# TaliMotzkin/GroupNet

Hardware: AMD Instinct MI355X
Metric: scenes/sec GroupNet MS-HGNN forward, NBA N=11 B=512, 1/2/4/8 MI355X (higher is better)
Workload: dtype f32

## Files before the change

groupnet_amd/_lib.py:

```python
from __future__ import annotations

import ctypes
import os
import threading

import torch

_HERE = os.path.dirname(os.path.abspath(__file__))
LIB_PATH = os.environ.get("GROUPNET_HIP_LIB") or os.path.join(_HERE, "libgroupnet_hip.so")
ABI_VERSION = 34

GN_OK = 0
GN_ERR_K_RANGE = -3

_P = ctypes.c_void_p
_I = ctypes.c_int
_F = ctypes.c_float
_SZ = ctypes.c_size_t
_U64 = ctypes.c_ulonglong


def addr(t) -> int:
    return 0 if t is None else t.data_ptr()


# ... 107 lines not shown
    "gn_listall_incidence_f32": (_I, [_P, _P, _I, _I, _I, _P]),
    "gn_affinity_topk_f32": (_I, [_P, _P, ctypes.POINTER(_P), ctypes.POINTER(_I), _I, _I, _I, _I,
                                  ctypes.POINTER(BlockExtras), _P]),
    "gn_affinity_topk_bf16": (_I, [_P, _P, ctypes.POINTER(_P), ctypes.POINTER(_I), _I, _I, _I, _I,
                                   ctypes.POINTER(BlockExtras), _P]),
    "gn_packed_elems": (_SZ, [_I, _I]),
    "gn_pack_linear_f32": (_I, [_P, _P, _I, _I, _I, _I, _P]),
    "gn_split_bf16_f32": (_I, [_P, _P, _I, _I, _P]),
    "gn_split_bf16_batch_f32": (_I, [_P, _I, _I, _I, _P]),
    "gn_pack_segments_f32": (_I, [_P, _I, _I, _P]),
    "gn_node_mlp_f32": (_I, [ctypes.POINTER(NodeGroup), _I, _I, _P]),
    "gn_node_mlp_bf16": (_I, [ctypes.POINTER(NodeGroup), _I, _I, _P]),
    "gn_node_mlp_affinity_f32": (_I, [ctypes.POINTER(NodeGroup), _I, _I, ctypes.POINTER(AffinityJob), _P]),
    "gn_node_mlp_affinity_bf16": (_I, [ctypes.POINTER(NodeGroup), _I, _I, ctypes.POINTER(AffinityJob), _P]),
    "gn_affinity_tail_lds_limit": (_SZ, []),
    "gn_node2edge_f32": (_I, [ctypes.POINTER(N2EGroup), _I, _I, _I, _P]),
    "gn_node2edge_bf16": (_I, [ctypes.POINTER(N2EGroup), _I, _I, _I, _P]),
    "gn_edge_mlp_gumbel_f32": (_I, [ctypes.POINTER(EdgeGroup), _I, _F, _U64, _P, _P]),
    "gn_edge_mlp_gumbel_bf16": (_I, [ctypes.POINTER(EdgeGroup), _I, _F, _U64, _P, _P]),
    "gn_agg_gather_f32": (_I, [ctypes.POINTER(GatherGroup), _I, _I, _I, _P]),
    "gn_agg_gather_bf16": (_I, [ctypes.POINTER(GatherGroup), _I, _I, _I, _P]),
    "gn_agg_mlp_f32": (_I, [ctypes.POINTER(AggGroup), _I, _P]),
    "gn_agg_mlp_bf16": (_I, [ctypes.POINTER(AggGroup), _I, _P]),
    "gn_node_linear_f32": (_I, [_P, _P, _P, _P, _I, _I, _P]),
    "gn_agg_scatter_f32": (_I, [ctypes.POINTER(ScatterGroup), _I, _I, _I, _F, _P]),
    "gn_agg_scatter_bf16": (_I, [ctypes.POINTER(ScatterGroup), _I, _I, _I, _F, _P]),
    "gn_mlp2_f32": (_I, [ctypes.POINTER(Mlp2Group), _I, _I, _I, _I, _I, _I, _I, _F, _P]),
    "gn_mlp2_bf16": (_I, [ctypes.POINTER(Mlp2Group), _I, _I, _I, _I, _I, _I, _I, _F, _P]),
    "gn_gemm_f32": (_I, [_P, _P, _P, _I, _I, _I, _I, _I, _I, _I, _I, _P, _P, _I, _I, _F, _F, _P]),
    "gn_gemm_grouped_f32": (_I, [ctypes.POINTER(GemmDesc), _I, _P]),
    "gn_typed_bwd_f32": (_I, [_P, _P, _P, _I, _P, _P, _P, ctypes.c_longlong, _I, _I, _P]),
    "gn_axpby2d_f32": (_I, [_P, _I, _P, _I, ctypes.c_longlong, _I, _F, _F, _P]),
    "gn_gumbel_ef_f32": (_I, [_P, _P, _P, ctypes.c_longlong, _I, _I, _I, _F, _I, _P]),
    "gn_gumbel_bwd_f32": (_I, [_P, _P, _P, _P, _P, ctypes.c_longlong, _I, _I, _F, _I, _P]),
# ... 51 lines not shown
```

groupnet_amd/csrc/gn_common.hpp:

```cpp
#pragma once
#include <hip/hip_runtime.h>
#include <stdint.h>
#include <stdlib.h>

#include "../../include/groupnet_hip.h"

#define GN_WAVE 64

typedef float f32x16 __attribute__((ext_vector_type(16)));
typedef float f32x4 __attribute__((ext_vector_type(4)));

static inline bool gn_aligned16(const void* p) { return (reinterpret_cast<uintptr_t>(p) & 15u) == 0; }

static inline int gn_check_launch() { return hipGetLastError() == hipSuccess ? GN_OK : GN_ERR_LAUNCH; }

#define GN_REQUIRE_PTR(p) \
  do {                    \
    if ((p) == nullptr) return GN_ERR_NULL; \
  } while (0)
#define GN_REQUIRE_ALIGNED(p) \
  do {                        \
    if (!gn_aligned16(p)) return GN_ERR_ALIGN; \
  } while (0)

__device__ __forceinline__ int gn_uniform(int v) { return __builtin_amdgcn_readfirstlane(v); }

__device__ __forceinline__ float gn_half_sum(float v) {
#pragma unroll
  for (int m = 16; m >= 1; m >>= 1) v += __shfl_xor(v, m, GN_WAVE);
  return v;
}
__device__ __forceinline__ float gn_wave_sum(float v) {
#pragma unroll
  for (int m = 32; m >= 1; m >>= 1) v += __shfl_xor(v, m, GN_WAVE);
  return v;
}
__device__ __forceinline__ float gn_wave_max(float v) {
#pragma unroll
  for (int m = 32; m >= 1; m >>= 1) v = fmaxf(v, __shfl_xor(v, m, GN_WAVE));
  return v;
// ... 98 lines not shown
```

groupnet_amd/csrc/gn_graph.hip:

```cpp
#include "gn_mlp_common.hpp"
#include "gn_affinity.hpp"

namespace {

constexpr int kBlock = 256;
constexpr int kN2EU = 4;
constexpr size_t kLdsBudget = 128 * 1024;

__device__ __forceinline__ bool beats(float vj, int j, float vc, int c) {
  const bool nj = vj != vj, nc = vc != vc;
  if (nj || nc) return (nj && !nc) || (nj && nc && j < c);
  return vj > vc || (vj == vc && j < c);
}

template <typename T>
__device__ __forceinline__ void emit_incidence(const float* row, int N, int b, int i, int c, const ScaleList& sl) {
  T* H_cat = reinterpret_cast<T*>(sl.H_cat);
  const float v = row[c];
  int rank = 0;
  for (int j = 0; j < N; ++j) rank += beats(row[j], j, v, c) ? 1 : 0;
  for (int s = 0; s < sl.n; ++s) {
    if (sl.k[s] == N) {
      if (i == 0) {
        sl.H[s][(size_t)b * N + c] = 1.f;
// ... 903 lines not shown
#pragma unroll
    for (int l = 0; l < 4; ++l) {
      const unsigned long long gidx = blk * 4 + l;
      if (gidx >= offset && gidx - offset < n) U[gidx - offset] = gn_philox_to_uniform(c[l]);
    }
  }
}

inline int capped_grid(long long work_items, int per_block, int cap = 256 * 16) {
  long long g = (work_items + per_block - 1) / per_block;
  return (int)(g < 1 ? 1 : (g > cap ? cap : g));
}

}

extern "C" int gn_abi_version(void) { return 34; }

extern "C" const char* gn_strerror(int code) {
  switch (code) {
    case GN_OK: return "ok";
    case GN_ERR_NULL: return "null pointer";
    case GN_ERR_SHAPE: return "unsupported or non-positive size";
    case GN_ERR_K_RANGE: return "selected index k out of range";
    case GN_ERR_ALIGN: return "pointer not 16-byte aligned";
    case GN_ERR_LAUNCH: return "kernel launch failed";
    case GN_ERR_LDS: return "tile does not fit in LDS";
    default: return "unknown error";
  }
}

extern "C" int gn_affinity_f32(const float* f, float* corr, int B, int N, int D, gn_stream_t stream) {
// ... 369 lines not shown
```

groupnet_amd/csrc/gn_mlp_bf16.hpp:

```cpp
#pragma once
#include "gn_mlp_common.hpp"
#include "gn_affinity.hpp"

#include <type_traits>

namespace {

constexpr int kOccP1 = 2;

template <int P>
struct Parts {
  bf16x8 p[P];
};

typedef float f32x8 __attribute__((ext_vector_type(8)));
__device__ __forceinline__ bf16x8 cvt_half(const f32x16& v, int hf) {
  f32x8 h;
#pragma unroll
  for (int jj = 0; jj < 8; ++jj) h[jj] = v[8 * hf + jj];
  return __builtin_convertvector(h, bf16x8);
}

typedef _Float16 f16x8 __attribute__((ext_vector_type(8)));
typedef _Float16 f16x2 __attribute__((ext_vector_type(2)));
// ... 62 lines not shown
constexpr int kMfmaPerSub = P == 3 ? 6 : (P == 2 ? 3 : 1);

template <int P, typename F>
__device__ __forceinline__ void run_with_fallback(F body) {
  ovf_t ovf = {0ull, 0};
  if constexpr (P == 2) {
    body(std::integral_constant<int, 2>{}, ovf);
    if (!__syncthreads_or(ovf.mask != 0ull || ovf.wf != 0)) return;
    ovf = {0ull, 0};
    body(std::integral_constant<int, 3>{}, ovf);
  } else {
    body(std::integral_constant<int, P>{}, ovf);
  }
}
__device__ __forceinline__ int image_flag(const void* image, int substeps) {
  return *reinterpret_cast<const int*>(reinterpret_cast<const char*>(image) + (size_t)substeps * 2 * 1024);
}
template <int P>
__device__ __forceinline__ const void* pick_image(const void* x, const void* h) { return P == 2 ? h : x; }

template <int P>
__device__ __forceinline__ void mfma_substep(const f32x4 (&w)[P], const Parts<P>& x, f32x16& acc) {
  if constexpr (P == 3) {
    const bf16x8 w1 = __builtin_bit_cast(bf16x8, w[0]);
    const bf16x8 w2 = __builtin_bit_cast(bf16x8, w[1]);
    const bf16x8 w3 = __builtin_bit_cast(bf16x8, w[2]);
    acc = __builtin_amdgcn_mfma_f32_32x32x16_bf16(w3, x.p[0], acc, 0, 0, 0);
    acc = __builtin_amdgcn_mfma_f32_32x32x16_bf16(w2, x.p[1], acc, 0, 0, 0);
    acc = __builtin_amdgcn_mfma_f32_32x32x16_bf16(w1, x.p[2], acc, 0, 0, 0);
    acc = __builtin_amdgcn_mfma_f32_32x32x16_bf16(w2, x.p[0], acc, 0, 0, 0);
    acc = __builtin_amdgcn_mfma_f32_32x32x16_bf16(w1, x.p[1], acc, 0, 0, 0);
// ... 111 lines not shown
    read_ops(s % CH + QD - 1, (s + QD - 1) % QD);
#pragma unroll
    for (int b = 0; b < RB; ++b) mfma_substep<P>(q[s % QD], x_of(b), acc_of(b));
    if constexpr (FENCE) __builtin_amdgcn_sched_barrier(0);
  }
  __device__ __forceinline__ void skip(int, int s, int n) {
#pragma unroll
    for (int p = s; p < s + n; ++p)
      if (p % CH == 0) boundary(p / CH);
    const int basec = (s + n - 1) / CH;
#pragma unroll
    for (int j = 0; j + 1 < QD; ++j) read_ops(s + n + j - basec * CH, (s + n + j) % QD);
  }
};

template <int P, int IT, int OT, int HT, bool PACKED_RELU = false, typename Stream, typename PostFn>
__device__ __forceinline__ void layer_pair(Stream& ws, int c0, int s0, const Parts<P> (&xi)[IT][2],
                                           const f32x16& hid0, const float* __restrict__ b0, int h,
                                           f32x16 (&out)[OT], ovf_t& ovf, PostFn post) {
  constexpr int NA = 2 * IT, NB = 2 * OT;
  constexpr int kMfma = NA * kMfmaPerSub<P>;
  constexpr int kValuPerPhase = P == 3 ? 96 : (P == 2 ? 84 : 40);
  constexpr int kValu = (kValuPerPhase + kMfma - 1) / kMfma;
  int pos = s0;
  f32x16 hidn = hid0;
  f32x16 bias_n;
  if (HT > 1) bias_n = load_bias_tile(b0 + 32, h);
#pragma unroll
  for (int u = 0; u < NA; ++u) {
    ws.step(c0, pos, xi[u >> 1][u & 1], hidn);
    ++pos;
  }
#pragma unroll
  for (int t = 0; t < HT; ++t) {
    f32x16 cur = hidn;
    if (t + 1 < HT) {
      hidn = bias_n;
      if (t + 2 < HT) bias_n = load_bias_tile(b0 + 32 * (t + 2), h);
    }
    post(t, cur);
    Parts<P> xh[2];
    if constexpr (PACKED_RELU) {
      make_parts_relu(cur, 0, xh[0]);
      make_parts_relu(cur, 1, xh[1]);
    } else {
      make_parts<P>(cur, 0, xh[0], ovf);
      make_parts<P>(cur, 1, xh[1], ovf);
    }
    if (t + 1 < HT) {
#pragma unroll
      for (int u = 0; u < NA; ++u) {
        ws.template step<false>(c0, pos, xi[u >> 1][u & 1], hidn);
        ++pos;
      }
#pragma unroll
      for (int i = 0; i < kMfma; ++i) {
        __builtin_amdgcn_sched_group_barrier(0x008, 1, 0);
        __builtin_amdgcn_sched_group_barrier(0x002, kValu, 0);
        if ((i % kMfmaPerSub<P>) == 0)
          __builtin_amdgcn_sched_group_barrier(Stream::CH == 1 ? 0x020 : 0x100, P, 0);
      }
    }
    __builtin_amdgcn_sched_barrier(0);
#pragma unroll
    for (int u = 0; u < NB; ++u) {
      ws.step(c0, pos, xh[u & 1], out[u >> 1]);
      ++pos;
    }
  }
}

template <typename T>
__device__ __forceinline__ void store_tile(T* __restrict__ p, const f32x16& a) {
#pragma unroll
  for (int q = 0; q < 4; ++q) {
    const f32x4 v = {a[4 * q + 0], a[4 * q + 1], a[4 * q + 2], a[4 * q + 3]};
    st4(p + 8 * q, v);
  }
// ... 82 lines not shown
#pragma unroll
    for (int oo = 0; oo < 4; ++oo) {
      const int o = o0 + o4 + oo;
      f32x16 acc = bn;
      bn = load_bias_tile(G.bA + 32 * min(o + 1, o0 + nt - 1), h);
#pragma unroll
      for (int i = 0; i < 4; ++i) ws.step(o4 * 4 / WS::CH, 4 * oo + i, xi[i >> 1][i & 1], acc);
      if (rb.live) store_tile(arow + 32 * o, acc);
    }
  }
}
template <int P>
constexpr int kRingF4For = WStream<P == 2 ? 3 : P>::kRingF4;

template <int P, typename T>
__global__ __launch_bounds__(256, 2) void node_stage_kernel(NodeTable Tb) {
  __shared__ f32x4 wring[kRingF4For<P>];
  if (Tb.aff_scenes > 0 && (int)blockIdx.x >= Tb.node_grid) {
    extern __shared__ __align__(16) float aff_lds[];
    affinity_topk_body<T>(reinterpret_cast<const T*>(Tb.aff_f), Tb.aff_corr, Tb.aff_sl, Tb.aff_N, Tb.aff_D, Tb.aff_ex,
                          (int)blockIdx.x - Tb.node_grid, aff_lds);
    return;
  }
  run_with_fallback<P>([&](auto pc, ovf_t& ovf) { node_stage_body<decltype(pc)::value, T>(Tb, wring, ovf); });
}

template <int P, typename T>
__device__ __forceinline__ void edge_x_body(const GroupTable<gn_edge_group_t>& Tb, float tau, unsigned long long seed,
                                            const unsigned long long* __restrict__ offset_dev, int pool_bytes,
                                            f32x4* wring, ovf_t& ovf) {
  using WS = WStream<P>;
  extern __shared__ __align__(16) unsigned char pool_dyn[];
  const int lwg = gn_uniform(gn_xcd_logical(Tb.xs, blockIdx.x));
  if (lwg < 0) return;
  const int gi = find_group(Tb, lwg);
  const gn_edge_group_t G = Tb.g[gi];
  const int rows = G.rows, K = G.K;
  const bool sparse = hyper_unstaged(G, 128, PoolStage<T>::kPitch * sizeof(T), pool_bytes);
  const int blk = sparse ? (wave_id() == 0 ? lwg - Tb.first_wg[gi] : (rows + 31) / 32) : (lwg - Tb.first_wg[gi]) * 4 + wave_id();
  const RowBlock rb = row_block(rows, blk);
  const int lane = rb.lane, h = rb.h;
  f32x16 in[2], z[2], lg;
  if (G.edges != nullptr) {
    load_rows<2>(reinterpret_cast<const T*>(G.edges), GN_FEAT, rb.row_ld, h, in);
  } else {
    const int nodes_max = G.pool_H == nullptr && G.sym_N > 0 ? pool_stage_nodes(128, gn_pair_count(G.pool_N), G.pool_N) : 0;
    const int r0 = (lwg - Tb.first_wg[gi]) * 128;
    if (G.pool_H != nullptr) {
      if (pool_bytes < 0)
        pooled_rows<T>(G, rb.row_ld, h, in);
      else if ((size_t)hyper_stage_nodes(128, G.pool_E, G.pool_N) * PoolStage<T>::kPitch * sizeof(T) <= (size_t)pool_bytes) {
        pooled_rows_hyper_staged<T, 1>(G, r0, min(rows - 1, r0 + 127), {rb.row_ld}, h, reinterpret_cast<T*>(pool_dyn),
                                       [&](auto, f32x16 (&p)[2]) { in[0] = p[0], in[1] = p[1]; });
      } else
        pooled_rows_hyper<T>(G, rb.row_ld, h, in);
    } else if (nodes_max > 0 && pool_bytes >= 0 && PoolStage<T>::bytes(nodes_max) <= (size_t)pool_bytes) {
      T* s_xp = reinterpret_cast<T*>(pool_dyn);
      T* s_pq = s_xp + (size_t)nodes_max * PoolStage<T>::kPitch;
      const int node0 = pool_stage_fill<T>(G, r0, min(rows - 1, r0 + 127), s_xp, s_pq);
      __syncthreads();
      pooled_rows_staged<T>(G, rb.row_ld, h, s_xp, s_pq, node0, in);
    } else {
      pooled_rows<T>(G, rb.row_ld, h, in);
    }
  }
  long long o1 = rb.row_ld, o2 = rb.row_ld;
  bool diag = true;
  if (G.sym_N > 0) {
    const int N = G.sym_N, Pn = gn_pair_count(N);
    const int b = rb.row_ld / Pn, p = rb.row_ld - b * Pn;
    int i, j;
    gn_pair_decode(p, N, i, j);
    o1 = (long long)b * N * N + i * N + j;
    o2 = (long long)b * N * N + j * N + i;
    diag = i == j;
  }
  float u1[8], u2[8];
  const unsigned long long pbase = G.philox_offset + (offset_dev ? *offset_dev : 0ull);
  const float* bi0 = G.bias;
  const float* bi1 = G.bias + 128;
  const float* bd0 = G.bias + 192;
  const float* bd1 = G.bias + 448;
  WS ws;
  const void* img = pick_image<P>(G.Wx, G.Wh);
  if constexpr (P == 2) ovf.wf |= image_flag(img, 80);
  ws.begin(img, wring, lane, wave_id(), 80 / WS::CH);
  const f32x16 hidA0 = load_bias_tile(bi0, h);
  z[0] = load_bias_tile(bi1, h);
  z[1] = load_bias_tile(bi1 + 32, h);
  Parts<P> xi[2][2];
  make_parts_tiles<P, 2>(in, xi, ovf);
  layer_pair<P, 2, 2, 4, P == 1>(ws, 0, 0, xi, hidA0, bi0, h, z, ovf, [&](int t, f32x16& hid) {
    if constexpr (P != 1) {
      relu16(hid);
      if (G.keep_z1 != nullptr && rb.live) store_tile(G.keep_z1 + (size_t)rb.row * 128 + 32 * t + 4 * h, hid);
    }
  });
  if (G.keep_z != nullptr) store_rows<2>(G.keep_z, GN_FEAT, rb.row, h, rb.live, z);
  const f32x16 hidB0 = load_bias_tile(bd0, h);
  f32x16 lgv[1];
  lgv[0] = load_bias_tile(bd1, h);
  make_parts_tiles<P, 2>(z, xi, ovf);
  layer_pair<P, 2, 1, 8, P == 1>(ws, 0, 32, xi, hidB0, bd0, h, lgv, ovf, [&](int t, f32x16& hid) {
    if constexpr (P != 1) {
      relu16(hid);
      if (G.keep_dh1 != nullptr && rb.live) store_tile(G.keep_dh1 + (size_t)rb.row * 256 + 32 * t + 4 * h, hid);
    }
  });
  lg = lgv[0];
  fetch_uniforms(G.U, pbase, seed, o1, K, h, u1);
  if (G.sym_N > 0) fetch_uniforms(G.U, pbase, seed, o2, K, h, u2);
  if (G.keep_lgf != nullptr && rb.live) store_tile(G.keep_lgf + (size_t)rb.row * 32 + 4 * h, lg);

  float facv = 0.f;
#pragma unroll
  for (int r = 0; r < 8; ++r)
    if (feat_of(r, h) == K) facv = lg[r];
  facv += __shfl_xor(facv, 32, GN_WAVE);
  const float sig = 1.f / (1.f + expf(-facv));
  float d1[8], d2[8];
  gumbel_softmax_row<P == 1>(lg, u1, K, tau, h, d1);
  if (G.sym_N > 0) gumbel_softmax_row<P == 1>(lg, u2, K, tau, h, d2);
  if (rb.live) {
    float* frow = G.edge_feat + (size_t)rb.row * K;
    T* dist = reinterpret_cast<T*>(G.dist);
    if (G.sym_N == 0) {
      T* drow = dist + (size_t)rb.row * K;
#pragma unroll
      for (int r = 0; r < 8; ++r) {
        const int f = feat_of(r, h);
        if (f < K) {
          st1(drow + f, d1[r]);
          frow[f] = sig * d1[r];
        }
      }
    } else {
#pragma unroll
      for (int r = 0; r < 8; ++r) {
        const int f = feat_of(r, h);
        if (f < K) {
          if (dist != nullptr) {
            st1(dist + (size_t)o1 * K + f, d1[r]);
            if (!diag) st1(dist + (size_t)o2 * K + f, d2[r]);
          }
          frow[f] = diag ? 2.f * (sig * d1[r]) : sig * d1[r] + sig * d2[r];
        }
      }
    }
  }
}
template <int P, typename T>
__global__ __launch_bounds__(256, P == 1 ? kOccP1 : 2) void edge_x_kernel(GroupTable<gn_edge_group_t> Tb, float tau,
                                                        unsigned long long seed,
                                                        const unsigned long long* __restrict__ offset_dev, int pool_bytes) {
  __shared__ f32x4 wring[kRingF4For<P>];
  run_with_fallback<P>([&](auto pc, ovf_t& ovf) {
    edge_x_body<decltype(pc)::value, T>(Tb, tau, seed, offset_dev, pool_bytes, wring, ovf);
  });
}

__device__ __forceinline__ void add_b2(const float* __restrict__ b2k, float efk, int lane, int h, f32x16 (&out)[2]) {
  const float f0 = h == 0 ? b2k[lane & 31] : 0.f;
  const float f1 = h == 0 ? b2k[32 + (lane & 31)] : 0.f;
  const float efb = h == 0 ? efk : 0.f;
  out[0] = __builtin_amdgcn_mfma_f32_32x32x2f32(f0, efb, out[0], 0, 0, 0);
  out[1] = __builtin_amdgcn_mfma_f32_32x32x2f32(f1, efb, out[1], 0, 0, 0);
}

__device__ __forceinline__ void add_b2_regs(float f0, float f1, float efk, int h, f32x16 (&out)[2]) {
  const float efb = h == 0 ? efk : 0.f;
// ... 1773 lines not shown
```

groupnet_amd/csrc/gn_mlp_common.hpp:

```cpp
#pragma once
#include <stdlib.h>

#include "gn_common.hpp"

namespace {

constexpr int kTileFloats = 32 * 32;

__device__ __forceinline__ constexpr int feat_of(int r, int h) { return (r & 3) + 8 * (r >> 2) + 4 * h; }

typedef __bf16 bf16x8 __attribute__((ext_vector_type(8)));
__device__ __forceinline__ void split3(float x, __bf16& p1, __bf16& p2, __bf16& p3) {
  p1 = (__bf16)x;
  const float r1 = x - (float)p1;
  p2 = (__bf16)r1;
  p3 = (__bf16)(r1 - (float)p2);
}

typedef __bf16 bf16x4 __attribute__((ext_vector_type(4)));
__device__ __forceinline__ f32x4 ld4(const float* p) { return *reinterpret_cast<const f32x4*>(p); }
__device__ __forceinline__ f32x4 ld4(const __bf16* p) {
  const bf16x4 v = *reinterpret_cast<const bf16x4*>(p);
  return f32x4{(float)v[0], (float)v[1], (float)v[2], (float)v[3]};
}
// ... 49 lines not shown
  return b;
}

__device__ __forceinline__ void relu16(f32x16& a) {
#pragma unroll
  for (int r = 0; r < 16; ++r) a[r] = fmaxf(a[r], 0.f);
}

struct RowBlock {
  int lane, h, row, row_ld;
  bool live;
};
__device__ __forceinline__ RowBlock row_block(int rows, int block_index) {
  RowBlock rb;
  rb.lane = threadIdx.x & 63;
  rb.h = rb.lane >> 5;
  rb.row = block_index * 32 + (rb.lane & 31);
  rb.live = rb.row < rows;
  rb.row_ld = rb.live ? rb.row : rows - 1;
  return rb;
}
__device__ __forceinline__ int wave_id() { return gn_uniform((int)(threadIdx.x >> 6)); }

template <typename G>
struct GroupTable {
  G g[GN_MAX_GROUPS];
  int first_wg[GN_MAX_GROUPS + 1];
  int n;
  XcdSections xs;
};
// ... 844 lines not shown
```

groupnet_amd/csrc/gn_mlp_mfma.hip:

```cpp
#include <stdlib.h>

#include "gn_mlp_common.hpp"
#include "gn_mlp_bf16.hpp"

namespace {


__global__ void pack_linear_kernel(const float* __restrict__ W, float* __restrict__ Wp, int out_f, int in_f,
                                   int ld, int col_off, int OT, int IT) {
  const size_t total = (size_t)OT * IT * kTileFloats;
  for (size_t idx = (size_t)blockIdx.x * blockDim.x + threadIdx.x; idx < total;
       idx += (size_t)gridDim.x * blockDim.x) {
    const int c = idx & 3;
    const int lane = (idx >> 2) & 63;
    const int q = (idx >> 8) & 3;
    const size_t tile = idx >> 10;
    const int t = (int)(tile % IT), o = (int)(tile / IT);
    const int row = 32 * o + (lane & 31);
    const int col = 32 * t + 8 * q + 4 * (lane >> 5) + c;
    Wp[idx] = (row < out_f && col < in_f) ? W[(size_t)row * ld + col_off + col] : 0.f;
  }
}

__global__ __launch_bounds__(256) void pack_segments_kernel(const gn_pack_seg_t* __restrict__ segs) {
// ... 737 lines not shown
  GN_REQUIRE_PTR(segs_dev);
  if (n_segs < 1 || n_segs > 65535 || max_elems < 1) return GN_ERR_SHAPE;
  int gx = (max_elems + 255) / 256;
  gx = gx > 16 ? 16 : gx;
  hipLaunchKernelGGL(pack_segments_kernel, dim3(gx, n_segs), dim3(256), 0, (hipStream_t)stream, segs_dev);
  return gn_check_launch();
}

template <typename G, typename F>
static int x_mode(const G* groups, int n, F has) {
  int cnt = 0;
  for (int g = 0; g < n; ++g) cnt += has(groups[g]) ? 1 : 0;
  return cnt == 0 ? 0 : (cnt == n ? 1 : -1);
}

constexpr size_t kAffTailLds = 24 * 1024;
template <int P, typename T>
static int node_stage_launch(const gn_node_group_t* groups, int n_groups, int rows, hipStream_t s,
                             const gn_affinity_job_t* job = nullptr) {
  NodeTable Tb{};
  Tb.n = n_groups;
  Tb.rows = rows;
  Tb.wgs_per_group = (rows + 127) / 128;
  Tb.chain_wgs = n_groups * Tb.wgs_per_group;
  int a_wgs = 0;
  for (int g = 0; g < n_groups; ++g) {
    const gn_node_group_t& G = groups[g];
    const void* ptrs[] = {G.x, G.Wx, G.bias, G.xp, G.pq};
    for (const void* p : ptrs) GN_CHECK(need(p, true));
    if (P == 1 && G.hid_out != nullptr) return GN_ERR_SHAPE;
    if (P == 2) GN_CHECK(need(G.Wh, true));
    Tb.a_first[g] = a_wgs;
    if (G.A != nullptr) {
      GN_CHECK(need(G.WAx, true));
// ... 24 lines not shown
    aff_lds = affinity_fused_lds(job->N, job->D, embed ? job->extras->x_dim : 0);
    if (aff_lds > kAffTailLds) return GN_ERR_LDS;
    if (job->extras != nullptr) {
      Tb.aff_ex = *job->extras;
      if (Tb.aff_ex.f_out != nullptr && (!gn_aligned16(Tb.aff_ex.f_out) || Tb.aff_ex.f_out_ld < job->D || (Tb.aff_ex.f_out_ld & 3)))
        return GN_ERR_ALIGN;
      Tb.aff_sl.H_cat = Tb.aff_ex.H_cat;
    }
    Tb.node_grid = node_grid;
    Tb.aff_scenes = job->B;
    Tb.aff_N = job->N;
    Tb.aff_D = job->D;
    Tb.aff_f = job->f;
    Tb.aff_corr = job->corr;
  }
  hipLaunchKernelGGL((node_stage_kernel<P, T>), dim3(node_grid + Tb.aff_scenes), dim3(256), aff_lds, s, Tb);
  return gn_check_launch();
}

extern "C" int gn_node_mlp_f32(const gn_node_group_t* groups, int n_groups, int rows, gn_stream_t stream) {
  GN_CHECK(check_groups(groups, n_groups));
  if (rows <= 0) return GN_ERR_SHAPE;
  const int xm = x_mode(groups, n_groups, [](const gn_node_group_t& G) { return G.Wx != nullptr; });
  if (xm < 0) return GN_ERR_SHAPE;
  if (xm == 1) {
    const int hm = x_mode(groups, n_groups, [](const gn_node_group_t& G) { return G.Wh != nullptr; });
    if (hm < 0) return GN_ERR_SHAPE;
    return hm ? node_stage_launch<2, float>(groups, n_groups, rows, (hipStream_t)stream)
              : node_stage_launch<3, float>(groups, n_groups, rows, (hipStream_t)stream);
  }
// ... 25 lines not shown
  GN_CHECK(check_groups(groups, n_groups));
  if (rows <= 0 || job == nullptr) return GN_ERR_SHAPE;
  if (x_mode(groups, n_groups, [](const gn_node_group_t& G) { return G.Wx != nullptr; }) != 1) return GN_ERR_SHAPE;
  const int hm = x_mode(groups, n_groups, [](const gn_node_group_t& G) { return G.Wh != nullptr; });
  if (hm < 0) return GN_ERR_SHAPE;
  return hm ? node_stage_launch<2, float>(groups, n_groups, rows, (hipStream_t)stream, job)
            : node_stage_launch<3, float>(groups, n_groups, rows, (hipStream_t)stream, job);
}
extern "C" int gn_node_mlp_affinity_bf16(const gn_node_group_t* groups, int n_groups, int rows, const gn_affinity_job_t* job,
                                         gn_stream_t stream) {
  GN_CHECK(check_groups(groups, n_groups));
  if (rows <= 0 || job == nullptr) return GN_ERR_SHAPE;
  return node_stage_launch<1, __bf16>(groups, n_groups, rows, (hipStream_t)stream, job);
}
extern "C" size_t gn_affinity_tail_lds_limit(void) { return kAffTailLds; }

static long long rb2_min_pairs() {
  if (const char* e = getenv("GN_RB2_MIN_PAIRS")) {
    const long long v = atoll(e);
    if (v > 0) return v;
  }
  return 2048;
}

constexpr size_t kEdgeCuLds = 160 * 1024;
template <typename K>
static size_t static_lds_of(K kernel) {
  hipFuncAttributes a{};
  return hipFuncGetAttributes(&a, reinterpret_cast<const void*>(kernel)) == hipSuccess ? a.sharedSizeBytes : kEdgeCuLds / 2;
}
static int edge_launch(const gn_edge_group_t* groups, int n_groups, float tau, unsigned long long seed,
                       const unsigned long long* offset_dev, hipStream_t stream, bool twin) {
  GN_CHECK(check_groups(groups, n_groups));
  if (!(tau > 0.f)) return GN_ERR_SHAPE;
  const int xm = x_mode(groups, n_groups, [](const gn_edge_group_t& G) { return G.Wx != nullptr; });
  if (xm < 0 || (twin && xm != 1)) return GN_ERR_SHAPE;
  GroupTable<gn_edge_group_t> T{};
  T.n = n_groups;
  int wg = 0;
  for (int g = 0; g < n_groups; ++g) {
    const gn_edge_group_t& G = groups[g];
    if (G.edges != nullptr) {
      GN_CHECK(need(G.edges, true));
    } else {
      if (!xm || G.keep_z1 || G.keep_z || G.keep_dh1 || G.keep_lgf) return GN_ERR_NULL;
      GN_CHECK(need(G.xp, true));
      GN_CHECK(need(G.pq, true));
// ... 8 lines not shown
      }
    }
    GN_CHECK(need(xm ? G.Wx : (const void*)G.W, true));
    GN_CHECK(need(G.bias, true));
    GN_CHECK(need(G.edge_feat, false));
    if (G.sym_N == 0) GN_CHECK(need(G.dist, false));
    if (G.rows <= 0 || G.K < 1 || G.K > 15 || G.sym_N < 0) return GN_ERR_SHAPE;
    if (G.sym_N > 0 && G.rows % gn_pair_count(G.sym_N) != 0) return GN_ERR_SHAPE;
    if (twin && (G.keep_z1 || G.keep_z || G.keep_dh1 || G.keep_lgf)) return GN_ERR_SHAPE;
    T.g[g] = G;
    T.first_wg[g] = wg;
    wg += row_grid(G.rows);
  }
  T.first_wg[n_groups] = wg;
  const bool no_pool_stage = getenv("GN_POOL_STAGE") != nullptr && atoi(getenv("GN_POOL_STAGE")) == 0;
  auto pool_bytes_for = [&](int wg_rows, size_t static_lds) -> int {
    if (no_pool_stage) return -1;
    const size_t cap = kEdgeCuLds / 2 - min(static_lds, kEdgeCuLds / 2);
    size_t need = 0;
    for (int g = 0; g < n_groups; ++g) {
      const gn_edge_group_t& G = groups[g];
      if (G.edges != nullptr || (G.pool_H == nullptr && G.sym_N <= 0)) continue;
      const size_t row_bytes = twin ? PoolStage<__bf16>::kPitch * sizeof(__bf16) : PoolStage<float>::kPitch * sizeof(float);
      const size_t b = G.pool_H != nullptr ? (size_t)hyper_stage_nodes(wg_rows, G.pool_E, G.pool_N) * row_bytes
                                           : 2 * (size_t)pool_stage_nodes(wg_rows, gn_pair_count(G.pool_N), G.pool_N) * row_bytes;
      if (b <= cap && b > need) need = b;
    }
    return (int)need;
  };
  auto launch_lds = [](int pb) { return (size_t)(pb > 0 ? pb : 0); };
  auto sparse_grid = [&](int pb, size_t row_bytes) {
    int w = 0;
    for (int g = 0; g < n_groups; ++g) {
      T.first_wg[g] = w;
      w += hyper_unstaged(groups[g], 128, row_bytes, pb) ? (groups[g].rows + 31) / 32 : row_grid(groups[g].rows);
    }
    T.first_wg[n_groups] = w;
  };
  if (twin) {
    long long pairs = 0;
    for (int g = 0; g < n_groups; ++g) pairs += ((groups[g].rows + 31) / 32 + 1) / 2;
    bool rb2 = pairs >= rb2_min_pairs();
    if (const char* e = getenv("GN_EDGE_RB2")) rb2 = atoi(e) != 0;
    if (rb2) {
      wg = 0;
      for (int g = 0; g < n_groups; ++g) {
        T.first_wg[g] = wg;
        wg += ((groups[g].rows + 31) / 32 + 7) / 8;
      }
      T.first_wg[n_groups] = wg;
      static const size_t rb2_static = static_lds_of(edge_rb2_kernel<__bf16>);
      const int pb = pool_bytes_for(256, rb2_static);
      hipLaunchKernelGGL((edge_rb2_kernel<__bf16>), dim3(table_xcd_grid(T)), dim3(256), launch_lds(pb), stream, T, tau, seed,
                         offset_dev, pb);
      return gn_check_launch();
    }
    static const size_t x1_static = static_lds_of(edge_x_kernel<1, __bf16>);
    const int pb = pool_bytes_for(128, x1_static);
    sparse_grid(pb, PoolStage<__bf16>::kPitch * sizeof(__bf16));
    hipLaunchKernelGGL((edge_x_kernel<1, __bf16>), dim3(table_xcd_grid(T)), dim3(256), launch_lds(pb), stream, T, tau, seed,
                       offset_dev, pb);
  }
  else if (xm) {
    const int hm = x_mode(groups, n_groups, [](const gn_edge_group_t& G) { return G.Wh != nullptr; });
    if (hm < 0) return GN_ERR_SHAPE;
    static const size_t x2_static = static_lds_of(edge_x_kernel<2, float>), x3_static = static_lds_of(edge_x_kernel<3, float>);
    const int pb = pool_bytes_for(128, hm ? x2_static : x3_static);
    sparse_grid(pb, PoolStage<float>::kPitch * sizeof(float));
    if (hm)
      hipLaunchKernelGGL((edge_x_kernel<2, float>), dim3(table_xcd_grid(T)), dim3(256), launch_lds(pb), stream, T, tau, seed,
                         offset_dev, pb);
    else
      hipLaunchKernelGGL((edge_x_kernel<3, float>), dim3(table_xcd_grid(T)), dim3(256), launch_lds(pb), stream, T, tau, seed,
                         offset_dev, pb);
  }
  else
    hipLaunchKernelGGL(edge_mlp_gumbel_kernel, dim3(wg), dim3(256), 0, stream, T, tau, seed, offset_dev);
  return gn_check_launch();
}
extern "C" int gn_edge_mlp_gumbel_f32(const gn_edge_group_t* groups, int n_groups, float tau,
                                      unsigned long long seed, const unsigned long long* offset_dev,
                                      gn_stream_t stream) {
  return edge_launch(groups, n_groups, tau, seed, offset_dev, (hipStream_t)stream, false);
}
extern "C" int gn_edge_mlp_gumbel_bf16(const gn_edge_group_t* groups, int n_groups, float tau,
                                       unsigned long long seed, const unsigned long long* offset_dev,
                                       gn_stream_t stream) {
  return edge_launch(groups, n_groups, tau, seed, offset_dev, (hipStream_t)stream, true);
}

static int agg_launch(const gn_agg_group_t* groups_in, int n_groups_in, hipStream_t stream, bool twin) {
  GN_CHECK(check_groups(groups_in, n_groups_in));
  gn_agg_group_t rest[GN_MAX_GROUPS];
  int n_groups = 0;
  for (int g = 0; g < n_groups_in; ++g) {
    const gn_agg_group_t& G = groups_in[g];
    if (!(G.node_form && G.A == nullptr)) {
      rest[n_groups++] = G;
// ... 305 lines not shown
```

include/groupnet_hip.h:

```cpp
#ifndef GROUPNET_HIP_H
#define GROUPNET_HIP_H

#include <stddef.h>

#ifdef __cplusplus
extern "C" {
#endif

typedef void* gn_stream_t;

#define GN_OK 0
#define GN_ERR_NULL -1
#define GN_ERR_SHAPE -2
#define GN_ERR_K_RANGE -3
#define GN_ERR_ALIGN -4
#define GN_ERR_LAUNCH -5
#define GN_ERR_LDS -6

#define GN_FEAT 64
#define GN_MAX_TYPES 16
#define GN_MAX_SCALES 8

int gn_copy_2d(void* dst, size_t dst_pitch, const void* src, size_t src_pitch, size_t width_bytes, int rows,
               gn_stream_t stream);
// ... 61 lines not shown
int gn_node_mlp_bf16(const gn_node_group_t* groups, int n_groups, int rows, gn_stream_t stream);
typedef struct {
  const void* f;
  float* corr;
  float* const* H_list;
  const int* k_list;
  int n_scales;
  int B, N, D;
  const gn_block_extras_t* extras;
} gn_affinity_job_t;
int gn_node_mlp_affinity_f32(const gn_node_group_t* groups, int n_groups, int rows, const gn_affinity_job_t* job,
                             gn_stream_t stream);
int gn_node_mlp_affinity_bf16(const gn_node_group_t* groups, int n_groups, int rows, const gn_affinity_job_t* job,
                              gn_stream_t stream);
size_t gn_affinity_tail_lds_limit(void);

typedef struct {
  const float* xp;
  const float* pq;
  const float* H;
  const float* w2;
  float* edges;
  const float* b2;
  int E;
  int sym;
} gn_n2e_group_t;
int gn_node2edge_f32(const gn_n2e_group_t* groups, int n_groups, int B, int N, gn_stream_t stream);
int gn_node2edge_bf16(const gn_n2e_group_t* groups, int n_groups, int B, int N, gn_stream_t stream);

typedef struct {
// ... 13 lines not shown
  float* keep_lgf;
  const void* Wx;
  const float* xp;
  const float* pq;
  const float* pool_H;
  const float* w2;
  const float* b2;
  int pool_N;
  int pool_E;
  const void* Wh;
} gn_edge_group_t;
int gn_edge_mlp_gumbel_f32(const gn_edge_group_t* groups, int n_groups, float tau, unsigned long long seed,
                           const unsigned long long* offset_dev, gn_stream_t stream);
int gn_edge_mlp_gumbel_bf16(const gn_edge_group_t* groups, int n_groups, float tau, unsigned long long seed,
                            const unsigned long long* offset_dev, gn_stream_t stream);

typedef struct {
  const float* ori;
  const float* H;
  float* eo;
  int E;
  int sym;
} gn_gather_group_t;
int gn_agg_gather_f32(const gn_gather_group_t* groups, int n_groups, int B, int N, gn_stream_t stream);
int gn_agg_gather_bf16(const gn_gather_group_t* groups, int n_groups, int B, int N, gn_stream_t stream);

typedef struct {
  const float* eo;
  const float* edge_feat;
  const float* W;
// ... 139 lines not shown
```

Baseline: 7.253 million.

## Raise node/edge MLP kernel occupancy by sharing LDS ring and recomputing row indices

Raises launch_bounds occupancy for the P=2 node and edge kernels to 3 workgroups per CU. To fit, the edge kernel's weight ring moves into dynamic LDS and the pool staging buffer reuses it, with added barriers. Row-block indices are recomputed late instead of kept live, the bias prefetch is delayed, and scalar uniform loads are used, all to cut register pressure. New launch-info queries report dynamic LDS and occupancy, at the risk of register spills or an LDS cap that disables pool staging.

```diff
diff --git a/groupnet_amd/_lib.py b/groupnet_amd/_lib.py
--- a/groupnet_amd/_lib.py
+++ b/groupnet_amd/_lib.py
@@ -8,7 +8,7 @@
 
 _HERE = os.path.dirname(os.path.abspath(__file__))
 LIB_PATH = os.environ.get("GROUPNET_HIP_LIB") or os.path.join(_HERE, "libgroupnet_hip.so")
-ABI_VERSION = 34
+ABI_VERSION = 35
 
 GN_OK = 0
 GN_ERR_K_RANGE = -3
@@ -146,10 +146,13 @@
     "gn_node_mlp_affinity_f32": (_I, [ctypes.POINTER(NodeGroup), _I, _I, ctypes.POINTER(AffinityJob), _P]),
     "gn_node_mlp_affinity_bf16": (_I, [ctypes.POINTER(NodeGroup), _I, _I, ctypes.POINTER(AffinityJob), _P]),
     "gn_affinity_tail_lds_limit": (_SZ, []),
+    "gn_node_mlp_affinity_launch_info_f32": (_I, [ctypes.POINTER(NodeGroup), _I, _I, ctypes.POINTER(AffinityJob),
+                                                  ctypes.POINTER(_SZ), ctypes.POINTER(_I)]),
     "gn_node2edge_f32": (_I, [ctypes.POINTER(N2EGroup), _I, _I, _I, _P]),
     "gn_node2edge_bf16": (_I, [ctypes.POINTER(N2EGroup), _I, _I, _I, _P]),
     "gn_edge_mlp_gumbel_f32": (_I, [ctypes.POINTER(EdgeGroup), _I, _F, _U64, _P, _P]),
     "gn_edge_mlp_gumbel_bf16": (_I, [ctypes.POINTER(EdgeGroup), _I, _F, _U64, _P, _P]),
+    "gn_edge_mlp_gumbel_launch_info_f32": (_I, [ctypes.POINTER(EdgeGroup), _I, ctypes.POINTER(_SZ), ctypes.POINTER(_I)]),
     "gn_agg_gather_f32": (_I, [ctypes.POINTER(GatherGroup), _I, _I, _I, _P]),
     "gn_agg_gather_bf16": (_I, [ctypes.POINTER(GatherGroup), _I, _I, _I, _P]),
     "gn_agg_mlp_f32": (_I, [ctypes.POINTER(AggGroup), _I, _P]),
diff --git a/groupnet_amd/csrc/gn_common.hpp b/groupnet_amd/csrc/gn_common.hpp
--- a/groupnet_amd/csrc/gn_common.hpp
+++ b/groupnet_amd/csrc/gn_common.hpp
@@ -24,6 +24,10 @@
   } while (0)
 
 __device__ __forceinline__ int gn_uniform(int v) { return __builtin_amdgcn_readfirstlane(v); }
+template <typename T>
+__device__ __forceinline__ T gn_uniform_load(const T* p) {
+  return *(const __attribute__((address_space(4))) T*)p;
+}
 
 __device__ __forceinline__ float gn_half_sum(float v) {
 #pragma unroll
diff --git a/groupnet_amd/csrc/gn_graph.hip b/groupnet_amd/csrc/gn_graph.hip
--- a/groupnet_amd/csrc/gn_graph.hip
+++ b/groupnet_amd/csrc/gn_graph.hip
@@ -941,7 +941,7 @@
 
 }
 
-extern "C" int gn_abi_version(void) { return 34; }
+extern "C" int gn_abi_version(void) { return 35; }
 
 extern "C" const char* gn_strerror(int code) {
   switch (code) {
diff --git a/groupnet_amd/csrc/gn_mlp_bf16.hpp b/groupnet_amd/csrc/gn_mlp_bf16.hpp
--- a/groupnet_amd/csrc/gn_mlp_bf16.hpp
+++ b/groupnet_amd/csrc/gn_mlp_bf16.hpp
@@ -7,6 +7,10 @@
 namespace {
 
 constexpr int kOccP1 = 2;
+template <int P>
+constexpr int kNodeOcc = P == 2 ? 3 : 2;
+template <int P>
+constexpr int kEdgeOcc = P == 1 ? kOccP1 : (P == 2 ? 3 : 2);
 
 template <int P>
 struct Parts {
@@ -100,7 +104,7 @@
   }
 }
 __device__ __forceinline__ int image_flag(const void* image, int substeps) {
-  return *reinterpret_cast<const int*>(reinterpret_cast<const char*>(image) + (size_t)substeps * 2 * 1024);
+  return gn_uniform_load(reinterpret_cast<const int*>(reinterpret_cast<const char*>(image) + (size_t)substeps * 2 * 1024));
 }
 template <int P>
 __device__ __forceinline__ const void* pick_image(const void* x, const void* h) { return P == 2 ? h : x; }
@@ -242,7 +246,7 @@
   }
 };
 
-template <int P, int IT, int OT, int HT, bool PACKED_RELU = false, typename Stream, typename PostFn>
+template <int P, int IT, int OT, int HT, bool PACKED_RELU = false, bool LATE_BIAS = false, typename Stream, typename PostFn>
 __device__ __forceinline__ void layer_pair(Stream& ws, int c0, int s0, const Parts<P> (&xi)[IT][2],
                                            const f32x16& hid0, const float* __restrict__ b0, int h,
                                            f32x16 (&out)[OT], ovf_t& ovf, PostFn post) {
@@ -264,7 +268,7 @@
     f32x16 cur = hidn;
     if (t + 1 < HT) {
       hidn = bias_n;
-      if (t + 2 < HT) bias_n = load_bias_tile(b0 + 32 * (t + 2), h);
+      if (!LATE_BIAS && t + 2 < HT) bias_n = load_bias_tile(b0 + 32 * (t + 2), h);
     }
     post(t, cur);
     Parts<P> xh[2];
@@ -290,6 +294,7 @@
       }
     }
     __builtin_amdgcn_sched_barrier(0);
+    if (LATE_BIAS && t + 2 < HT) bias_n = load_bias_tile(b0 + 32 * (t + 2), h);
 #pragma unroll
     for (int u = 0; u < NB; ++u) {
       ws.step(c0, pos, xh[u & 1], out[u >> 1]);
@@ -402,7 +407,7 @@
 constexpr int kRingF4For = WStream<P == 2 ? 3 : P>::kRingF4;
 
 template <int P, typename T>
-__global__ __launch_bounds__(256, 2) void node_stage_kernel(NodeTable Tb) {
+__global__ __launch_bounds__(256, kNodeOcc<P>) void node_stage_kernel(NodeTable Tb) {
   __shared__ f32x4 wring[kRingF4For<P>];
   if (Tb.aff_scenes > 0 && (int)blockIdx.x >= Tb.node_grid) {
     extern __shared__ __align__(16) float aff_lds[];
@@ -418,7 +423,7 @@
                                             const unsigned long long* __restrict__ offset_dev, int pool_bytes,
                                             f32x4* wring, ovf_t& ovf) {
   using WS = WStream<P>;
-  extern __shared__ __align__(16) unsigned char pool_dyn[];
+  unsigned char* pool_dyn = reinterpret_cast<unsigned char*>(wring);
   const int lwg = gn_uniform(gn_xcd_logical(Tb.xs, blockIdx.x));
   if (lwg < 0) return;
   const int gi = find_group(Tb, lwg);
@@ -440,6 +445,7 @@
       else if ((size_t)hyper_stage_nodes(128, G.pool_E, G.pool_N) * PoolStage<T>::kPitch * sizeof(T) <= (size_t)pool_bytes) {
         pooled_rows_hyper_staged<T, 1>(G, r0, min(rows - 1, r0 + 127), {rb.row_ld}, h, reinterpret_cast<T*>(pool_dyn),
                                        [&](auto, f32x16 (&p)[2]) { in[0] = p[0], in[1] = p[1]; });
+        __syncthreads();
       } else
         pooled_rows_hyper<T>(G, rb.row_ld, h, in);
     } else if (nodes_max > 0 && pool_bytes >= 0 && PoolStage<T>::bytes(nodes_max) <= (size_t)pool_bytes) {
@@ -448,23 +454,13 @@
       const int node0 = pool_stage_fill<T>(G, r0, min(rows - 1, r0 + 127), s_xp, s_pq);
       __syncthreads();
       pooled_rows_staged<T>(G, rb.row_ld, h, s_xp, s_pq, node0, in);
+      __syncthreads();
     } else {
       pooled_rows<T>(G, rb.row_ld, h, in);
     }
   }
-  long long o1 = rb.row_ld, o2 = rb.row_ld;
-  bool diag = true;
-  if (G.sym_N > 0) {
-    const int N = G.sym_N, Pn = gn_pair_count(N);
-    const int b = rb.row_ld / Pn, p = rb.row_ld - b * Pn;
-    int i, j;
-    gn_pair_decode(p, N, i, j);
-    o1 = (long long)b * N * N + i * N + j;
-    o2 = (long long)b * N * N + j * N + i;
-    diag = i == j;
-  }
   float u1[8], u2[8];
-  const unsigned long long pbase = G.philox_offset + (offset_dev ? *offset_dev : 0ull);
+  const unsigned long long pbase = G.philox_offset + (offset_dev ? gn_uniform_load(offset_dev) : 0ull);
   const float* bi0 = G.bias;
   const float* bi1 = G.bias + 128;
   const float* bd0 = G.bias + 192;
@@ -478,13 +474,19 @@
   z[1] = load_bias_tile(bi1 + 32, h);
   Parts<P> xi[2][2];
   make_parts_tiles<P, 2>(in, xi, ovf);
-  layer_pair<P, 2, 2, 4, P == 1>(ws, 0, 0, xi, hidA0, bi0, h, z, ovf, [&](int t, f32x16& hid) {
+  layer_pair<P, 2, 2, 4, P == 1, P == 2>(ws, 0, 0, xi, hidA0, bi0, h, z, ovf, [&](int t, f32x16& hid) {
     if constexpr (P != 1) {
       relu16(hid);
-      if (G.keep_z1 != nullptr && rb.live) store_tile(G.keep_z1 + (size_t)rb.row * 128 + 32 * t + 4 * h, hid);
+      if (G.keep_z1 != nullptr) {
+        const RowBlock rk = row_block_again(rows, blk);
+        if (rk.live) store_tile(G.keep_z1 + (size_t)rk.row * 128 + 32 * t + 4 * h, hid);
+      }
     }
   });
-  if (G.keep_z != nullptr) store_rows<2>(G.keep_z, GN_FEAT, rb.row, h, rb.live, z);
+  if (G.keep_z != nullptr) {
+    const RowBlock rk = row_block_again(rows, blk);
+    store_rows<2>(G.keep_z, GN_FEAT, rk.row, h, rk.live, z);
+  }
   const f32x16 hidB0 = load_bias_tile(bd0, h);
   f32x16 lgv[1];
   lgv[0] = load_bias_tile(bd1, h);
@@ -492,13 +494,28 @@
   layer_pair<P, 2, 1, 8, P == 1>(ws, 0, 32, xi, hidB0, bd0, h, lgv, ovf, [&](int t, f32x16& hid) {
     if constexpr (P != 1) {
       relu16(hid);
-      if (G.keep_dh1 != nullptr && rb.live) store_tile(G.keep_dh1 + (size_t)rb.row * 256 + 32 * t + 4 * h, hid);
+      if (G.keep_dh1 != nullptr) {
+        const RowBlock rk = row_block_again(rows, blk);
+        if (rk.live) store_tile(G.keep_dh1 + (size_t)rk.row * 256 + 32 * t + 4 * h, hid);
+      }
     }
   });
   lg = lgv[0];
+  const RowBlock re = row_block_again(rows, blk);
+  long long o1 = re.row_ld, o2 = re.row_ld;
+  bool diag = true;
+  if (G.sym_N > 0) {
+    const int N = G.sym_N, Pn = gn_pair_count(N);
+    const int b = re.row_ld / Pn, p = re.row_ld - b * Pn;
+    int i, j;
+    gn_pair_decode(p, N, i, j);
+    o1 = (long long)b * N * N + i * N + j;
+    o2 = (long long)b * N * N + j * N + i;
+    diag = i == j;
+  }
   fetch_uniforms(G.U, pbase, seed, o1, K, h, u1);
   if (G.sym_N > 0) fetch_uniforms(G.U, pbase, seed, o2, K, h, u2);
-  if (G.keep_lgf != nullptr && rb.live) store_tile(G.keep_lgf + (size_t)rb.row * 32 + 4 * h, lg);
+  if (G.keep_lgf != nullptr && re.live) store_tile(G.keep_lgf + (size_t)re.row * 32 + 4 * h, lg);
 
   float facv = 0.f;
 #pragma unroll
@@ -509,11 +526,11 @@
   float d1[8], d2[8];
   gumbel_softmax_row<P == 1>(lg, u1, K, tau, h, d1);
   if (G.sym_N > 0) gumbel_softmax_row<P == 1>(lg, u2, K, tau, h, d2);
-  if (rb.live) {
-    float* frow = G.edge_feat + (size_t)rb.row * K;
+  if (re.live) {
+    float* frow = G.edge_feat + (size_t)re.row * K;
     T* dist = reinterpret_cast<T*>(G.dist);
     if (G.sym_N == 0) {
-      T* drow = dist + (size_t)rb.row * K;
+      T* drow = dist + (size_t)re.row * K;
 #pragma unroll
       for (int r = 0; r < 8; ++r) {
         const int f = feat_of(r, h);
@@ -538,10 +555,11 @@
   }
 }
 template <int P, typename T>
-__global__ __launch_bounds__(256, P == 1 ? kOccP1 : 2) void edge_x_kernel(GroupTable<gn_edge_group_t> Tb, float tau,
+__global__ __launch_bounds__(256, kEdgeOcc<P>) void edge_x_kernel(GroupTable<gn_edge_group_t> Tb, float tau,
                                                         unsigned long long seed,
                                                         const unsigned long long* __restrict__ offset_dev, int pool_bytes) {
-  __shared__ f32x4 wring[kRingF4For<P>];
+  extern __shared__ __align__(16) unsigned char ring_and_stage[];
+  f32x4* wring = reinterpret_cast<f32x4*>(ring_and_stage);
   run_with_fallback<P>([&](auto pc, ovf_t& ovf) {
     edge_x_body<decltype(pc)::value, T>(Tb, tau, seed, offset_dev, pool_bytes, wring, ovf);
   });
diff --git a/groupnet_amd/csrc/gn_mlp_common.hpp b/groupnet_amd/csrc/gn_mlp_common.hpp
--- a/groupnet_amd/csrc/gn_mlp_common.hpp
+++ b/groupnet_amd/csrc/gn_mlp_common.hpp
@@ -87,6 +87,17 @@
 __device__ __forceinline__ RowBlock row_block(int rows, int block_index) {
   RowBlock rb;
   rb.lane = threadIdx.x & 63;
+  rb.h = rb.lane >> 5;
+  rb.row = block_index * 32 + (rb.lane & 31);
+  rb.live = rb.row < rows;
+  rb.row_ld = rb.live ? rb.row : rows - 1;
+  return rb;
+}
+__device__ __forceinline__ RowBlock row_block_again(int rows, int block_index) {
+  int t = threadIdx.x;
+  asm volatile("" : "+v"(t));
+  RowBlock rb;
+  rb.lane = t & 63;
   rb.h = rb.lane >> 5;
   rb.row = block_index * 32 + (rb.lane & 31);
   rb.live = rb.row < rows;
diff --git a/groupnet_amd/csrc/gn_mlp_mfma.hip b/groupnet_amd/csrc/gn_mlp_mfma.hip
--- a/groupnet_amd/csrc/gn_mlp_mfma.hip
+++ b/groupnet_amd/csrc/gn_mlp_mfma.hip
@@ -775,10 +775,22 @@
   return cnt == 0 ? 0 : (cnt == n ? 1 : -1);
 }
 
+struct LaunchQuery {
+  size_t* dyn_lds;
+  int* wgs_per_cu;
+  template <typename K>
+  int fill(K kernel, size_t lds) const {
+    *dyn_lds = lds;
+    return hipOccupancyMaxActiveBlocksPerMultiprocessor(wgs_per_cu, reinterpret_cast<const void*>(kernel), 256, lds) == hipSuccess
+               ? GN_OK
+               : GN_ERR_LAUNCH;
+  }
+};
+
 constexpr size_t kAffTailLds = 24 * 1024;
 template <int P, typename T>
 static int node_stage_launch(const gn_node_group_t* groups, int n_groups, int rows, hipStream_t s,
-                             const gn_affinity_job_t* job = nullptr) {
+                             const gn_affinity_job_t* job = nullptr, LaunchQuery* query = nullptr) {
   NodeTable Tb{};
   Tb.n = n_groups;
   Tb.rows = rows;
@@ -833,6 +845,7 @@
     Tb.aff_f = job->f;
     Tb.aff_corr = job->corr;
   }
+  if (query != nullptr) return query->fill(node_stage_kernel<P, T>, aff_lds);
   hipLaunchKernelGGL((node_stage_kernel<P, T>), dim3(node_grid + Tb.aff_scenes), dim3(256), aff_lds, s, Tb);
   return gn_check_launch();
 }
@@ -888,6 +901,18 @@
   return node_stage_launch<1, __bf16>(groups, n_groups, rows, (hipStream_t)stream, job);
 }
 extern "C" size_t gn_affinity_tail_lds_limit(void) { return kAffTailLds; }
+extern "C" int gn_node_mlp_affinity_launch_info_f32(const gn_node_group_t* groups, int n_groups, int rows,
+                                                    const gn_affinity_job_t* job, size_t* dyn_lds, int* wgs_per_cu) {
+  GN_CHECK(check_groups(groups, n_groups));
+  if (dyn_lds == nullptr || wgs_per_cu == nullptr) return GN_ERR_NULL;
+  if (rows <= 0 || job == nullptr) return GN_ERR_SHAPE;
+  if (x_mode(groups, n_groups, [](const gn_node_group_t& G) { return G.Wx != nullptr; }) != 1) return GN_ERR_SHAPE;
+  const int hm = x_mode(groups, n_groups, [](const gn_node_group_t& G) { return G.Wh != nullptr; });
+  if (hm < 0) return GN_ERR_SHAPE;
+  LaunchQuery q{dyn_lds, wgs_per_cu};
+  return hm ? node_stage_launch<2, float>(groups, n_groups, rows, nullptr, job, &q)
+            : node_stage_launch<3, float>(groups, n_groups, rows, nullptr, job, &q);
+}
 
 static long long rb2_min_pairs() {
   if (const char* e = getenv("GN_RB2_MIN_PAIRS")) {
@@ -898,13 +923,16 @@
 }
 
 constexpr size_t kEdgeCuLds = 160 * 1024;
+constexpr size_t kLdsGranule = 1280;
+template <int P>
+constexpr size_t kEdgeRing = kRingF4For<P> * sizeof(f32x4);
 template <typename K>
 static size_t static_lds_of(K kernel) {
   hipFuncAttributes a{};
   return hipFuncGetAttributes(&a, reinterpret_cast<const void*>(kernel)) == hipSuccess ? a.sharedSizeBytes : kEdgeCuLds / 2;
 }
 static int edge_launch(const gn_edge_group_t* groups, int n_groups, float tau, unsigned long long seed,
-                       const unsigned long long* offset_dev, hipStream_t stream, bool twin) {
+                       const unsigned long long* offset_dev, hipStream_t stream, bool twin, const LaunchQuery* query = nullptr) {
   GN_CHECK(check_groups(groups, n_groups));
   if (!(tau > 0.f)) return GN_ERR_SHAPE;
   const int xm = x_mode(groups, n_groups, [](const gn_edge_group_t& G) { return G.Wx != nullptr; });
@@ -943,10 +971,11 @@
   }
   T.first_wg[n_groups] = wg;
   const bool no_pool_stage = getenv("GN_POOL_STAGE") != nullptr && atoi(getenv("GN_POOL_STAGE")) == 0;
-  auto pool_bytes_for = [&](int wg_rows, size_t static_lds) -> int {
+  auto pool_bytes_for = [&](int wg_rows, size_t static_lds, int occ, size_t ring) -> int {
     if (no_pool_stage) return -1;
-    const size_t cap = kEdgeCuLds / 2 - min(static_lds, kEdgeCuLds / 2);
-    size_t need = 0;
+    const size_t share = kEdgeCuLds / occ / kLdsGranule * kLdsGranule;
+    const size_t cap = min(share - min(static_lds, share), (size_t)64 * 1024);
+    size_t need = ring;
     for (int g = 0; g < n_groups; ++g) {
       const gn_edge_group_t& G = groups[g];
       if (G.edges != nullptr || (G.pool_H == nullptr && G.sym_N <= 0)) continue;
@@ -957,7 +986,7 @@
     }
     return (int)need;
   };
-  auto launch_lds = [](int pb) { return (size_t)(pb > 0 ? pb : 0); };
+  auto launch_lds = [](int pb, size_t ring) { return pb > 0 ? (size_t)pb : ring; };
   auto sparse_grid = [&](int pb, size_t row_bytes) {
     int w = 0;
     for (int g = 0; g < n_groups; ++g) {
@@ -979,29 +1008,31 @@
       }
       T.first_wg[n_groups] = wg;
       static const size_t rb2_static = static_lds_of(edge_rb2_kernel<__bf16>);
-      const int pb = pool_bytes_for(256, rb2_static);
-      hipLaunchKernelGGL((edge_rb2_kernel<__bf16>), dim3(table_xcd_grid(T)), dim3(256), launch_lds(pb), stream, T, tau, seed,
+      const int pb = pool_bytes_for(256, rb2_static, 2, 0);
+      hipLaunchKernelGGL((edge_rb2_kernel<__bf16>), dim3(table_xcd_grid(T)), dim3(256), launch_lds(pb, 0), stream, T, tau, seed,
                          offset_dev, pb);
       return gn_check_launch();
     }
     static const size_t x1_static = static_lds_of(edge_x_kernel<1, __bf16>);
-    const int pb = pool_bytes_for(128, x1_static);
+    const int pb = pool_bytes_for(128, x1_static, kEdgeOcc<1>, kEdgeRing<1>);
     sparse_grid(pb, PoolStage<__bf16>::kPitch * sizeof(__bf16));
-    hipLaunchKernelGGL((edge_x_kernel<1, __bf16>), dim3(table_xcd_grid(T)), dim3(256), launch_lds(pb), stream, T, tau, seed,
+    hipLaunchKernelGGL((edge_x_kernel<1, __bf16>), dim3(table_xcd_grid(T)), dim3(256), launch_lds(pb, kEdgeRing<1>), stream, T, tau, seed,
                        offset_dev, pb);
   }
   else if (xm) {
     const int hm = x_mode(groups, n_groups, [](const gn_edge_group_t& G) { return G.Wh != nullptr; });
     if (hm < 0) return GN_ERR_SHAPE;
     static const size_t x2_static = static_lds_of(edge_x_kernel<2, float>), x3_static = static_lds_of(edge_x_kernel<3, float>);
-    const int pb = pool_bytes_for(128, hm ? x2_static : x3_static);
+    const int pb = hm ? pool_bytes_for(128, x2_static, kEdgeOcc<2>, kEdgeRing<2>) : pool_bytes_for(128, x3_static, kEdgeOcc<3>, kEdgeRing<3>);
     sparse_grid(pb, PoolStage<float>::kPitch * sizeof(float));
+    if (query != nullptr)
+      return hm ? query->fill(edge_x_kernel<2, float>, launch_lds(pb, kEdgeRing<2>)) : query->fill(edge_x_kernel<3, float>, launch_lds(pb, kEdgeRing<3>));
     if (hm)
-      hipLaunchKernelGGL((edge_x_kernel<2, float>), dim3(table_xcd_grid(T)), dim3(256), launch_lds(pb), stream, T, tau, seed,
-                         offset_dev, pb);
+      hipLaunchKernelGGL((edge_x_kernel<2, float>), dim3(table_xcd_grid(T)), dim3(256), launch_lds(pb, kEdgeRing<2>), stream, T, tau,
+                         seed, offset_dev, pb);
     else
-      hipLaunchKernelGGL((edge_x_kernel<3, float>), dim3(table_xcd_grid(T)), dim3(256), launch_lds(pb), stream, T, tau, seed,
-                         offset_dev, pb);
+      hipLaunchKernelGGL((edge_x_kernel<3, float>), dim3(table_xcd_grid(T)), dim3(256), launch_lds(pb, kEdgeRing<3>), stream, T, tau,
+                         seed, offset_dev, pb);
   }
   else
     hipLaunchKernelGGL(edge_mlp_gumbel_kernel, dim3(wg), dim3(256), 0, stream, T, tau, seed, offset_dev);
@@ -1011,6 +1042,13 @@
                                       unsigned long long seed, const unsigned long long* offset_dev,
                                       gn_stream_t stream) {
   return edge_launch(groups, n_groups, tau, seed, offset_dev, (hipStream_t)stream, false);
+}
+extern "C" int gn_edge_mlp_gumbel_launch_info_f32(const gn_edge_group_t* groups, int n_groups, size_t* dyn_lds, int* wgs_per_cu) {
+  GN_CHECK(check_groups(groups, n_groups));
+  if (dyn_lds == nullptr || wgs_per_cu == nullptr) return GN_ERR_NULL;
+  if (x_mode(groups, n_groups, [](const gn_edge_group_t& G) { return G.Wx != nullptr; }) != 1) return GN_ERR_SHAPE;
+  const LaunchQuery q{dyn_lds, wgs_per_cu};
+  return edge_launch(groups, n_groups, 1.f, 0ull, nullptr, nullptr, false, &q);
 }
 extern "C" int gn_edge_mlp_gumbel_bf16(const gn_edge_group_t* groups, int n_groups, float tau,
                                        unsigned long long seed, const unsigned long long* offset_dev,
diff --git a/include/groupnet_hip.h b/include/groupnet_hip.h
--- a/include/groupnet_hip.h
+++ b/include/groupnet_hip.h
@@ -99,6 +99,8 @@
 int gn_node_mlp_affinity_bf16(const gn_node_group_t* groups, int n_groups, int rows, const gn_affinity_job_t* job,
                               gn_stream_t stream);
 size_t gn_affinity_tail_lds_limit(void);
+int gn_node_mlp_affinity_launch_info_f32(const gn_node_group_t* groups, int n_groups, int rows, const gn_affinity_job_t* job,
+                                         size_t* dyn_lds, int* wgs_per_cu);
 
 typedef struct {
   const float* xp;
@@ -142,6 +144,7 @@
                            const unsigned long long* offset_dev, gn_stream_t stream);
 int gn_edge_mlp_gumbel_bf16(const gn_edge_group_t* groups, int n_groups, float tau, unsigned long long seed,
                             const unsigned long long* offset_dev, gn_stream_t stream);
+int gn_edge_mlp_gumbel_launch_info_f32(const gn_edge_group_t* groups, int n_groups, size_t* dyn_lds, int* wgs_per_cu);
 
 typedef struct {
   const float* ori;
```

Measured after the change: 7.472 million, median of 6. 3.0% higher.
